# Isomorpfishm/SINGA

Hardware: AMD Instinct MI355X
Metric: protein-ligand graphs/sec GAN step (G+D fwd+bwd); scatter-TP kernel HBM GB/s (higher is better)
Workload: dtype f32

## Files before the change

### __graft_entry__.py

```python
import os
import subprocess
import sys

ROOT = os.path.dirname(os.path.abspath(__file__))
if ROOT not in sys.path:
    sys.path.insert(0, ROOT)

SRC = os.path.join(ROOT, "singa_amd", "csrc", "singa_hip.hip")
LIB = os.path.join(ROOT, "singa_amd", "lib", "libsinga_hip.so")


def build() -> None:
    os.makedirs(os.path.dirname(LIB), exist_ok=True)
    deps = [SRC, os.path.join(ROOT, "singa_amd", "csrc", "so3_index.h"), os.path.join(ROOT, "include", "singa_hip.h"),
            os.path.join(ROOT, "include", "singa_hip_lab.h"), os.path.join(ROOT, "include", "singa_hip_gen.h"),
            os.path.join(ROOT, "include", "singa_hip_force.h"), os.path.join(ROOT, "include", "singa_hip_swor.h"),
            os.path.join(ROOT, "include", "singa_hip_stream.h"), os.path.join(ROOT, "include", "singa_hip_valence.h"),
            os.path.join(ROOT, "include", "singa_hip_beam.h"), os.path.join(ROOT, "include", "singa_hip_units.h"),
            os.path.join(ROOT, "include", "singa_hip_prefix.h"), os.path.join(ROOT, "include", "singa_hip_data.h")]
    if not os.path.exists(LIB) or any(os.path.getmtime(d) > os.path.getmtime(LIB) for d in deps):
        hipcc = os.environ.get("HIPCC", "/opt/rocm/bin/hipcc")
        cmd = [hipcc, "--offload-arch=gfx950", "-O3", "-std=c++17", "-shared", "-fPIC", "-o", LIB, SRC]
        subprocess.check_call(cmd)
    import torch
    import singa_amd
    from singa_amd import _capi
    _capi.bind(LIB)


def smoke() -> None:
    import numpy as np
    import torch

    build()
    from oracle import singa_oracle as O
    from singa_amd import graph as G
    from singa_amd.config import load_config
    from singa_amd.model.GAN import SINGA
    from tests.helpers import golden, state_from_spec

    assert torch.cuda.is_available(), "smoke() needs a GPU"
    L = 2
    dev = "cuda:0"
    sd = state_from_spec(f"singa_L{L}")
    z = golden(f"singa_L{L}_B3.npz")
    names = ["3wi2_4tpp", "4agq_5a7b", "5cp5_4nue"]
    batch = G.collate([G.load_npz(os.path.join(ROOT, "tests", "golden", f"graph_{n}.npz"), with_lap=False) for n in names])
    batch.nodes[G.PA]["lap_pe"], batch.nodes[G.LA]["lap_pe"] = torch.tensor(z["lap_p"]), torch.tensor(z["lap_l"])
    batch.extras["edge_rot_mat"] = {k: torch.tensor(z[f"rot_{k}"]) for k in ("pp", "ll", "lp")}
    batch.extras["knn"] = {G.PA: torch.tensor(z["knn_p"]), G.LA: torch.tensor(z["knn_l"])}
    batch = batch.to(dev)
    model = SINGA(load_config(lmax=L), device=dev)
    model.load_state_dict(sd, strict=False)
    model.eval()
    logits = model(batch)
    loss = torch.nn.functional.cross_entropy(logits, batch["ligand_data"]["smiIndices_tgt"].reshape(-1))
    loss.backward()
    torch.cuda.synchronize()
    og = O.collate([O.load_graph_npz(os.path.join(ROOT, "tests", "golden", f"graph_{n}.npz")) for n in names])
    rots = {k: torch.as_tensor(z[f"rot_{k}"]) for k in ("pp", "ll", "lp")}
    with torch.no_grad():
        ref = O.singa_forward(sd, og, rots, L, torch.as_tensor(z["knn_p"]), torch.as_tensor(z["knn_l"]),
                              torch.as_tensor(z["lap_p"]), torch.as_tensor(z["lap_l"]))
    err = float((logits.detach().cpu().double() - ref.double()).norm() / ref.double().norm())
    gn = float(torch.sqrt(sum((p.grad.double() ** 2).sum() for p in model.parameters() if p.grad is not None)))
    print(f"smoke: loss {float(loss):.6f} (reference {float(z['loss']):.6f}), logits rel err vs oracle {err:.2e}, "
          f"grad norm {gn:.4f} (reference {float(z['grad_total']):.4f})")
    assert err < 1e-4, err
    assert abs(gn - float(z["grad_total"])) < 1e-4 * float(z["grad_total"])


if __name__ == "__main__":
# ... 4 lines not shown
```

### singa_amd/_capi.py

```python
import ctypes as C

P = C.c_void_p
I32 = C.c_int
I64 = C.c_int64
F32 = C.c_float


class Seg(C.Structure):
    _fields_ = [("ptr", P), ("ld", I64), ("rows", C.c_int32)]


SegArr = Seg * 3


class Gemm(C.Structure):
    _fields_ = [("a", P), ("b", P), ("c", P), ("bias", P), ("lda", I64), ("ldb", I64), ("ldc", I64), ("I", C.c_int32),
                ("J", C.c_int32), ("R", C.c_int32), ("a_group", C.c_int32), ("b_group", C.c_int32), ("c_group", C.c_int32),
                ("a_group_ld", I64), ("b_group_ld", I64), ("c_group_ld", I64), ("c_split_stride", I64), ("mask", P),
                ("addend", P), ("relu", C.c_int32), ("asum", P), ("asum_stride", I64)]


class CGemm(C.Structure):
    _fields_ = [("a", P), ("b", P), ("c", P), ("lda", I64), ("ldb", I64), ("ldc", I64), ("a_im", I64), ("b_im", I64),
                ("c_im", I64), ("c_split_stride", I64), ("I", C.c_int32), ("J", C.c_int32), ("R", C.c_int32),
# ... 117 lines not shown
_SWOR_SIGS = {
    "singa_swor_noise_host": ([U64, P, P, P, I32, P, P, P], I32),
    "singa_swor_work": ([I32, I32], C.c_longlong),
    "singa_swor_expand": ([P, P, P, P, I32, I32, I32, I32, I32, F32, U64, P, I32] + [P] * 8 + [P], I32),
    "singa_swor_select": ([P, P, P, P, P, I32, I32, I32, I32, I32, I32, I32] + [P] * 13 + [P], I32),
    "singa_swor_follow": ([P] * 8 + [I32] * 6 + [I64] * 4 + [P], I32),
}
SWOR_EXPORTS = tuple(_SWOR_SIGS)

_STREAM_SIGS = {
    "singa_dec_self_attn_rows": ([P] * 10 + [I32, I32, P, F32, P], I32),
    "singa_sample_token_stream": ([P] * 6 + [I32, I32, I32, I32, I32, F32, I32, F32, I32, I32] + [P] * 7 + [P], I32),
    "singa_stream_refill": ([I32] * 8 + [P] * 8 + [P], I32),
    "singa_stream_refill_host": ([I32] * 8 + [P] * 8, I32),
}
STREAM_EXPORTS = tuple(_STREAM_SIGS)

_VALENCE_SIGS = {
    "singa_sample_token_valence": ([P] * 7 + [I32, I32, I32, I32, I32, F32, I32, F32, I32, I32] + [P] * 12 + [P], I32),
    "singa_valence_rule_host": ([P] * 5 + [I32] + [P] * 3, I32),
}
VALENCE_EXPORTS = tuple(_VALENCE_SIGS)

_BEAM_SIGS = {
    "singa_beam_work": ([I32, I32], C.c_longlong),
    "singa_beam_expand": ([P] * 5 + [I32] * 5 + [P] * 5 + [P], I32),
    "singa_beam_select": ([P] * 4 + [I32] * 7 + [P] * 18 + [P], I32),
}
BEAM_EXPORTS = tuple(_BEAM_SIGS)

_UNITS_SIGS = {
    "singa_edge_mlp_units_fwd": ([P] * 13 + [I32, I32, I32, I32, P], I32),
    "singa_edge_mlp_units_bwd": ([P] * 8 + [I32, I32, I32, P], I32),
}
UNITS_EXPORTS = tuple(_UNITS_SIGS)

_PREFIX_SIGS = {
    "singa_sample_token_stream_forced": ([P] * 7 + [I32, I32, I32, I32, I32, F32, I32, F32, I32, I32] + [P] * 10 + [P], I32),
    "singa_swor_expand_forced": ([P, P, P, P, I32, I32, I32, I32, I32, F32, U64, P, I32] + [P] * 9 + [P], I32),
    "singa_forced_beam_expand": ([P] * 5 + [I32] * 5 + [P] * 6 + [P], I32),
}
PREFIX_EXPORTS = tuple(_PREFIX_SIGS)


class CollateField(C.Structure):
    _fields_ = [("src", P), ("dst", P), ("axis", C.c_int32), ("width", C.c_int32), ("kind", C.c_int32), ("base_axis", C.c_int32)]


_DATA_SIGS = {
    "singa_collate_batch": ([P, I32, I32, P, P, P, C.POINTER(CollateField), I32, C.POINTER(I64), P], I32),
}
DATA_EXPORTS = tuple(_DATA_SIGS)


def bind(path):
    import torch
    lib = C.CDLL(path)
    for name, (args, res) in list(_SIGS.items()) + list(_LAB_SIGS.items()) + list(_GEN_SIGS.items()) + \
            list(_FORCE_SIGS.items()) + list(_SWOR_SIGS.items()) + list(_STREAM_SIGS.items()) + list(_VALENCE_SIGS.items()) + \
            list(_BEAM_SIGS.items()) + list(_UNITS_SIGS.items()) + list(_PREFIX_SIGS.items()) + list(_DATA_SIGS.items()):
        fn = getattr(lib, name)
        fn.argtypes = args
        fn.restype = res
    return lib


def segs(items):
    arr = SegArr()
    for i, (p, ld, rows) in enumerate(items):
        arr[i].ptr, arr[i].ld, arr[i].rows = p, ld, rows
    return arr, len(items)


def check(lib, code, what):
    if code != 0:
        raise RuntimeError(f"{what} failed ({code}): {lib.singa_last_error_string().decode()}")
```

### singa_amd/csrc/singa_hip.hip

```cpp
#include <hip/hip_runtime.h>
#include <hip/hip_ext.h>

#include <math.h>
#include <stdint.h>
#include <stdio.h>
#include <string.h>
#include <type_traits>

#include "../../include/singa_hip.h"
#include "../../include/singa_hip_lab.h"
#include "../../include/singa_hip_gen.h"
#include "../../include/singa_hip_force.h"
#include "../../include/singa_hip_swor.h"
#include "../../include/singa_hip_stream.h"
#include "../../include/singa_hip_valence.h"
#include "../../include/singa_hip_beam.h"
#include "../../include/singa_hip_units.h"
#include "../../include/singa_hip_prefix.h"
#include "../../include/singa_hip_data.h"
#include "so3_index.h"

namespace {

thread_local char g_err[256] = "ok";

int fail(int code, const char* msg) {
    snprintf(g_err, sizeof(g_err), "%s", msg);
    return code;
}

int check_launch(const char* what) {
    hipError_t e = hipGetLastError();
    if (e != hipSuccess) {
        snprintf(g_err, sizeof(g_err), "%s: %s", what, hipGetErrorString(e));
        return (int)e;
    }
    return SINGA_OK;
}

struct ProfRec {
    hipEvent_t a, b;
    int E, N, tag;
};
constexpr int PROF_CAP = 8192;
ProfRec g_prof[PROF_CAP];
int g_prof_n = 0;
bool g_prof_on = false;
unsigned long long* g_stamp_buf = nullptr;
int g_stamp_cap = 0;
__global__ void stamp_kernel(unsigned long long* dst) { *dst = (unsigned long long)wall_clock64(); }
int g_prof_edges_hint = 0;

#ifndef SINGA_KEEP_VGPR
#define SINGA_KEEP_VGPR(x) __asm__ volatile("" : "+v"(x))
#endif

#define SINGA_LAUNCH(tag_, E_, N_, kern, grid, block, st, ...)                                                   \
    do {                                                                                                          \
        if (g_prof_on && g_prof_n < PROF_CAP) {                                                                   \
            ProfRec& r_ = g_prof[g_prof_n++];                                                                     \
            (void)hipEventCreate(&r_.a);                                                                          \
            (void)hipEventCreate(&r_.b);                                                                          \
            r_.E = (E_);                                                                                          \
            r_.N = (N_);                                                                                          \
            r_.tag = (tag_);                                                                                      \
            hipExtLaunchKernelGGL(kern, grid, block, 0, (st), r_.a, r_.b, 0, __VA_ARGS__);                        \
        } else if (g_stamp_buf && 2 * (g_prof_n + 2) <= g_stamp_cap && g_prof_n + 1 < PROF_CAP) {                 \
            if (g_prof_n == 0) {                                                                                  \
                g_prof[0].a = g_prof[0].b = nullptr;                                                              \
                g_prof[0].E = g_prof[0].N = g_prof[0].tag = 0;                                                    \
// ... 859 lines not shown
#pragma unroll
        for (int h = 0; h < H; ++h) gn[h] = g[((long long)n * H + h) * F + f];
        const int beg = row_ptr[n], end = row_ptr[n + 1];
        for (int e = beg; e < end; e += 2) {
            const bool two = e + 1 < end;
            const int e1 = two ? e + 1 : e;
            const int j0 = col[e], j1 = col[e1];
            const float w0 = wv[(long long)e * F + f], w1 = wv[(long long)e1 * F + f];
            float t0[H], t1[H], gw0 = 0.f, gw1 = 0.f;
#pragma unroll
            for (int h = 0; h < H; ++h) {
                t0[h] = gn[h] * hv[((long long)j0 * H + h) * F + f];
                t1[h] = gn[h] * hv[((long long)j1 * H + h) * F + f];
            }
#pragma unroll
            for (int h = 0; h < H; ++h) {
                gw0 = fmaf(t0[h], alpha[(long long)e * H + h], gw0);
                gw1 = fmaf(t1[h], alpha[(long long)e1 * H + h], gw1);
            }
            const float p0 = quad_reduce4(t0[0] * w0, t0[1] * w0, t0[2] * w0, t0[3] * w0, f);
            const float p1 = quad_reduce4(t1[0] * w1, t1[1] * w1, t1[2] * w1, t1[3] * w1, f);
            if ((f & 15) == 0) {
                g_alpha[(long long)e * H + quarter] = p0;
                if (two) g_alpha[(long long)e1 * H + quarter] = p1;
            }
            g_wv[(long long)e * F + f] = gw0;
            if (two) g_wv[(long long)e1 * F + f] = gw1;
        }
    }
}

template <int H>
__global__ void __launch_bounds__(64) gather_wsum_bwd_col_kernel(const float* __restrict__ g, const float* __restrict__ alpha,
                                                                 const float* __restrict__ wv, const int* __restrict__ col_ptr,
                                                                 const int* __restrict__ eperm, const int* __restrict__ row,
                                                                 float* __restrict__ g_hv, int N) {
    constexpr int F = 64;
    const int f = threadIdx.x;
    SINGA_XCD_NODE_LOOP(j, N) {
        float acc[H];
#pragma unroll
        for (int h = 0; h < H; ++h) acc[h] = 0.f;
        const int beg = col_ptr[j], end = col_ptr[j + 1];
        for (int i = beg; i < end; ++i) {
            const int e = eperm[i];
            const int n = row[e];
            const float w = wv[(long long)e * F + f];
#pragma unroll
            for (int h = 0; h < H; ++h)
                acc[h] = fmaf(alpha[(long long)e * H + h] * w, g[((long long)n * H + h) * F + f], acc[h]);
        }
#pragma unroll
        for (int h = 0; h < H; ++h) g_hv[((long long)j * H + h) * F + f] = acc[h];
    }
}


template <int C>
__device__ __forceinline__ void ln_row(const float* __restrict__ x, long long r, float (&xh)[C], float& rstd, float eps) {
    float mean = 0.f;
#pragma unroll
    for (int c = 0; c < C; c += 4) {
        const float4 v = *reinterpret_cast<const float4*>(x + r * C + c);
        xh[c] = v.x, xh[c + 1] = v.y, xh[c + 2] = v.z, xh[c + 3] = v.w;
        mean += (v.x + v.y) + (v.z + v.w);
    }
    mean *= 1.f / C;
    float var = 0.f;
#pragma unroll
    for (int c = 0; c < C; ++c) {
        xh[c] -= mean;
        var = fmaf(xh[c], xh[c], var);
    }
    rstd = 1.f / sqrtf(var * (1.f / C) + eps);
#pragma unroll
    for (int c = 0; c < C; ++c) xh[c] *= rstd;
}

template <int C>
__global__ void __launch_bounds__(64) ln_silu_fwd_kernel(const float* __restrict__ x, const float* __restrict__ gamma,
                                                         const float* __restrict__ beta, float* __restrict__ out, long long M,
                                                         float eps) {
    const long long stride = (long long)gridDim.x * 64;
    for (long long r = (long long)blockIdx.x * 64 + threadIdx.x; r < M; r += stride) {
        float xh[C], rstd;
        ln_row<C>(x, r, xh, rstd, eps);
        float o[C];
#pragma unroll
        for (int c = 0; c < C; ++c) {
            const float y = fmaf(xh[c], gamma[c], beta[c]);
            o[c] = y / (1.f + expf(-y));
        }
#pragma unroll
        for (int c = 0; c < C; c += 4) *reinterpret_cast<float4*>(out + r * C + c) = make_float4(o[c], o[c + 1], o[c + 2], o[c + 3]);
    }
}

template <int C>
__global__ void __launch_bounds__(64) ln_silu_bwd_kernel(const float* __restrict__ x, const float* __restrict__ gamma,
                                                         const float* __restrict__ beta, const float* __restrict__ g_out,
                                                         float* __restrict__ g_x, float* __restrict__ part, long long M,
                                                         float eps) {
    const long long tid = (long long)blockIdx.x * 64 + threadIdx.x, stride = (long long)gridDim.x * 64;
    float ag[C], ab[C];
#pragma unroll
    for (int c = 0; c < C; ++c) ag[c] = ab[c] = 0.f;
// ... 5300 lines not shown
                                                       g_out, gx, g_gate, EC, G));
    return check_launch("s2act_bwd");
}

int singa_edge_logits_fwd(const float* qp, const float* wk, const float* hk, const float* cterm, const int32_t* row_ptr,
                          const int32_t* col, float* qk, int N, int H, int D, float scale, void* stream) {
    if (!qp || !wk || !hk || !cterm || !row_ptr || !col || !qk) return fail(SINGA_E_NULL, "edge_logits_fwd: null pointer");
    if (H != 4 || D != 32) return fail(SINGA_E_SHAPE, "edge_logits: built for H = 4 heads, D = 32 key channels per head");
    if (N <= 0) return SINGA_OK;
    hipLaunchKernelGGL((edge_logits_fwd_kernel<32, 4>), dim3(kn_grid(N)), dim3(64), 0, (hipStream_t)stream, qp, wk,
                       hk, cterm, row_ptr, col, qk, N, scale);
    return check_launch("edge_logits_fwd");
}

int singa_edge_logits_bwd(const float* g, const float* qp, const float* wk, const float* hk, const int32_t* row_ptr,
                          const int32_t* col, const int32_t* col_ptr, const int32_t* eperm, const int32_t* row,
                          float* g_qp, float* g_wk, float* g_hk, float* g_cterm, int N, int H, int D, float scale,
                          void* stream) {
    if (!g || !qp || !wk || !hk || !row_ptr || !col || !col_ptr || !eperm || !row || !g_qp || !g_wk || !g_hk || !g_cterm)
        return fail(SINGA_E_NULL, "edge_logits_bwd: null pointer");
    if (H != 4 || D != 32) return fail(SINGA_E_SHAPE, "edge_logits: built for H = 4 heads, D = 32 key channels per head");
    if (N <= 0) return SINGA_OK;
    hipLaunchKernelGGL((edge_logits_bwd_row_kernel<32, 4>), dim3(kn_grid(N)), dim3(64), 0, (hipStream_t)stream, g,
                       qp, wk, hk, row_ptr, col, g_qp, g_wk, g_cterm, N, scale);
    hipLaunchKernelGGL((edge_logits_bwd_col_kernel<32, 4>), dim3(kn_grid(N)), dim3(64), 0, (hipStream_t)stream, g,
                       qp, wk, col_ptr, eperm, row, g_hk, N, scale);
    return check_launch("edge_logits_bwd");
}

int singa_gather_wsum_fwd(const float* alpha, const float* wv, const float* hv, const int32_t* row_ptr, const int32_t* col,
                          float* out, int N, int H, int F, void* stream) {
    if (!alpha || !wv || !hv || !row_ptr || !col || !out) return fail(SINGA_E_NULL, "gather_wsum_fwd: null pointer");
    if (H != 4 || F != 64) return fail(SINGA_E_SHAPE, "gather_wsum: built for H = 4 heads, F = 64 value channels per head");
    if (N <= 0) return SINGA_OK;
    hipLaunchKernelGGL((gather_wsum_fwd_kernel<4>), dim3(kn_grid(N)), dim3(64), 0, (hipStream_t)stream, alpha, wv,
                       hv, row_ptr, col, out, N);
    return check_launch("gather_wsum_fwd");
}

int singa_gather_wsum_bwd(const float* g, const float* alpha, const float* wv, const float* hv, const int32_t* row_ptr,
                          const int32_t* col, const int32_t* col_ptr, const int32_t* eperm, const int32_t* row,
                          float* g_alpha, float* g_wv, float* g_hv, int N, int H, int F, void* stream) {
    if (!g || !alpha || !wv || !hv || !row_ptr || !col || !col_ptr || !eperm || !row || !g_alpha || !g_wv || !g_hv)
        return fail(SINGA_E_NULL, "gather_wsum_bwd: null pointer");
    if (H != 4 || F != 64) return fail(SINGA_E_SHAPE, "gather_wsum: built for H = 4 heads, F = 64 value channels per head");
    if (N <= 0) return SINGA_OK;
    hipLaunchKernelGGL((gather_wsum_bwd_row_kernel<4>), dim3(kn_grid(N)), dim3(64), 0, (hipStream_t)stream, g,
                       alpha, wv, hv, row_ptr, col, g_alpha, g_wv, N);
    hipLaunchKernelGGL((gather_wsum_bwd_col_kernel<4>), dim3(kn_grid(N)), dim3(64), 0, (hipStream_t)stream, g,
                       alpha, wv, col_ptr, eperm, row, g_hv, N);
    return check_launch("gather_wsum_bwd");
}

#define SINGA_DISPATCH_S2SEP(lmax, edge, ...)                                                            \
    do {                                                                                                 \
        if (edge) {                                                                                      \
            constexpr bool EDGE_ = true; constexpr int C_ = 128;                                         \
            switch (lmax) {                                                                              \
                case 2: { constexpr int L_ = 2; __VA_ARGS__; } break;                                    \
                case 4: { constexpr int L_ = 4; __VA_ARGS__; } break;                                    \
                case 6: { constexpr int L_ = 6; __VA_ARGS__; } break;                                    \
                default: return fail(SINGA_E_LMAX, "s2act_sep: lmax must be 2, 4 or 6");                 \
            }                                                                                            \
        } else {                                                                                         \
            constexpr bool EDGE_ = false; constexpr int C_ = 512;                                        \
            switch (lmax) {                                                                              \
                case 2: { constexpr int L_ = 2; __VA_ARGS__; } break;                                    \
                case 4: { constexpr int L_ = 4; __VA_ARGS__; } break;                                    \
                case 6: { constexpr int L_ = 6; __VA_ARGS__; } break;                                    \
                default: return fail(SINGA_E_LMAX, "s2act_sep: lmax must be 2, 4 or 6");                 \
            }                                                                                            \
        }                                                                                                \
    } while (0)

int singa_s2act_sep_fwd(const singa_seg_t* x, int nseg, const float* gate, int64_t ldg, const float* P, const float* Q,
                        const float* A, float* out, int E, int C, int lmax, void* stream) {
    Segs s;
    if (!pack(x, nseg, &s) || !gate || !P || !Q || !A || !out) return fail(SINGA_E_NULL, "s2act_sep_fwd: null pointer");
    const bool edge = nseg == 3;
    if (!(edge && C == 128) && !(nseg == 1 && C == 512))
        return fail(SINGA_E_SHAPE, "s2act_sep: built for (3 segments, C = 128) and (1 segment, C = 512)");
    if (edge && (s.rows[0] != lmax + 1 || s.rows[1] != 2 * lmax || s.rows[2] != 2 * (lmax - 1)))
        return fail(SINGA_E_SHAPE, "s2act_sep(edge): segment rows must be L+1, 2L, 2(L-1)");
    if (!edge && s.rows[0] != (lmax + 1) * (lmax + 1)) return fail(SINGA_E_SHAPE, "s2act_sep(node): rows must be (L+1)^2");
    if (E <= 0) return SINGA_OK;
    long long EC = (long long)E * C;
    int blocks = (int)((EC + 255) / 256);
    const int tag = edge ? SINGA_PROF_S2_EDGE_FWD : SINGA_PROF_S2_NODE_FWD;
    bool pair = (((uintptr_t)gate | (uintptr_t)out) & 7) == 0 && ldg % 2 == 0 && (edge || lmax <= 4);
    for (int i = 0; i < nseg; ++i) pair = pair && ((uintptr_t)s.p[i] & 7) == 0 && s.ld[i] % 2 == 0;
    if (pair) {
        const long long EC2 = EC / 2;
        blocks = (int)((EC2 + 255) / 256);
        SINGA_DISPATCH_S2SEP(lmax, edge, SINGA_LAUNCH(tag, E, 0, (s2act_sep_fwd2_kernel<L_, EDGE_, C_>), dim3(blocks), dim3(256),
                                                      (hipStream_t)stream, s, gate, (long long)ldg, P, Q, out, EC2));
        return check_launch("s2act_sep_fwd");
    }
    SINGA_DISPATCH_S2SEP(lmax, edge, SINGA_LAUNCH(tag, E, 0, (s2act_sep_fwd_kernel<L_, EDGE_, C_>), dim3(blocks), dim3(256),
                                                  (hipStream_t)stream, s, gate, (long long)ldg, P, Q, A, out, EC));
    return check_launch("s2act_sep_fwd");
}

int singa_s2act_sep_bwd_seg(const singa_seg_t* x, int nseg, const float* gate, int64_t ldg, const float* P, const float* Q,
                            const float* A, const float* g_out, const singa_seg_mut_t* gx, float* g_gate, int64_t ld_gg, int E,
                            int C, int lmax, void* stream) {
    Segs s;
// ... 1383 lines not shown
```

### singa_amd/model/CProMG.py

```python
import math
import os

import numpy as np
import torch
import torch.nn as nn
import torch.nn.functional as F
from torch.nn import BatchNorm1d, Conv1d, Dropout, Embedding, LayerNorm, Sequential

from .. import ops
from ..nn import Linear


class ShiftedSoftplus(nn.Module):
    def __init__(self, device="cuda"):
        super().__init__()
        self.shift = math.log(2.0)

    def forward(self, x):
        return F.softplus(x) - self.shift


class GaussianSmearing(nn.Module):
    def __init__(self, start=0.0, stop=10.0, num_gaussians=50, device="cuda"):
        super().__init__()
# ... 68 lines not shown
                  else torch.zeros((), dtype=torch.bool, device=dev))
        n_groups, last, triple = torch.stack([gid[-1] + 1, skey[-1], triple.to(gid.dtype)]).tolist()
        n_edges = n_groups - (1 if last == sentinel else 0)
        ukey = torch.zeros(n_groups, dtype=torch.int64, device=dev).scatter_(0, gid, skey)[:n_edges]
        ln2 = torch.cat([ln, ln])[perm]
        if not triple:
            nxt = torch.cat([ln2[1:], ln2[-1:]])
            prv = torch.cat([ln2[:1], ln2[:-1]])
            has_next = torch.cat([~new[1:], new.new_zeros(1)])
            mean = torch.where(new, torch.where(has_next, 0.5 * (ln2 + nxt), ln2), 0.5 * (prv + ln2))
            ln = torch.zeros(n_groups, device=dev).scatter_(0, gid, mean)[:n_edges]
        else:
            cnt = torch.zeros(n_groups, device=dev).index_add_(0, gid, torch.ones_like(ln2))[:n_edges]
            ln = torch.zeros(n_groups, device=dev).index_add_(0, gid, ln2)[:n_edges] / cnt
        row, col = ukey // N, ukey % N
        fused = ln.is_cuda and smear.offset.numel() == 64
        ea = None if fused else smear(ln)
        self.n_edges = n_edges + N
        if cap is not None:
            extra = cap - self.n_edges
            nd = N - n_real
            if extra < 0 or nd < 2:
                raise OverflowError(f"KnnEdges: {self.n_edges} edges do not fit the capacity {cap}")
            i = torch.arange(extra, device=dev)
            ps = (i * nd) // max(extra, 1)
            row = torch.cat([row, n_real + ps])
            col = torch.cat([col, n_real + (ps + 1 + i % (nd - 1)) % nd])
            if not fused:
                ea = torch.cat([ea, ea.new_zeros(extra, ea.shape[1])])
        loop = torch.arange(N, device=dev)
        bounds = torch.arange(N + 1, device=dev)
        if ln.is_cuda:
            E0 = row.shape[0]
            seg_ptr = torch.searchsorted(row, bounds)
            order = torch.empty(E0 + N, dtype=torch.int64, device=dev)
            order[torch.arange(E0, device=dev) + row] = torch.arange(E0, device=dev)
            order[seg_ptr[1:] + loop] = E0 + loop
            row, col = torch.cat([row, loop]), torch.cat([col, loop])
            self.row, self.col = row[order], col[order]
            seg32 = seg_ptr.to(torch.int32)
            if fused:
                self.attr = ops.knn_edge_attr(ln, seg32, E0, n_edges, smear.offset, smear.coeff)
            else:
                deg = ops.segment_sum_rows(ea.contiguous(), seg32)
                self.attr = torch.cat([-ea, deg], 0)[order].contiguous()
        else:
            deg = torch.zeros(N, ea.shape[1], device=dev).index_add_(0, row, ea)
            row, col = torch.cat([row, loop]), torch.cat([col, loop])
            attr = torch.cat([-ea, deg], 0)
            order = torch.argsort(row, stable=True)
            self.row, self.col, self.attr = row[order], col[order], attr[order].contiguous()
        self.row_ptr = torch.searchsorted(self.row, bounds).to(torch.int32)
        self.row32, self.col32 = self.row.to(torch.int32), self.col.to(torch.int32)
        eperm = torch.argsort(self.col32 if ln.is_cuda else self.col, stable=True)
        self.eperm = eperm.to(torch.int32)
        self.col_ptr = torch.searchsorted(self.col[eperm], bounds).to(torch.int32)
        self.N = N
        self.unit_a, self.unit_b = self._units(ukey, n_real, bool(triple))

    def _units(self, ukey, n_real, repeats):
        row, col = self.row, self.col
        E, N = row.shape[0], self.N
        idx = torch.arange(E, device=row.device)
        if repeats or ukey.numel() == 0:
            single = torch.ones_like(row, dtype=torch.bool)
        else:
            single = row == col
            if n_real is not None:
                single |= torch.maximum(row, col) >= n_real
        mate = torch.where(single, idx, torch.searchsorted(ukey, col * N + row) + col)
        first = single | (row < col)
        slot = torch.where(first, torch.cumsum(first, 0) - 1, E)
        both = torch.stack([idx, mate], 1).to(torch.int32)
        units = torch.full((E + 1, 2), -1, dtype=torch.int32, device=row.device).index_copy_(0, slot, both)
        return units[:E, 0].contiguous(), units[:E, 1].contiguous()

    def tensors(self):
        return [self.row, self.col, self.attr, self.row_ptr, self.row32, self.col32, self.eperm, self.col_ptr, self.unit_a,
                self.unit_b]


class MultiHeadAttention(nn.Module):

    def __init__(self, hidden_channels, edge_channels, key_channels, num_heads=1, device="cuda"):
        super().__init__()
        assert hidden_channels % num_heads == 0 and key_channels % num_heads == 0
        self.num_heads = num_heads
        self.k_lin = Conv1d(hidden_channels, key_channels, 1, groups=num_heads, bias=False, device=device)
        self.q_lin = Conv1d(hidden_channels, key_channels, 1, groups=num_heads, bias=False, device=device)
        self.v_lin = Conv1d(hidden_channels, hidden_channels, 1, groups=num_heads, bias=False, device=device)
        kh, vh = key_channels // num_heads, hidden_channels // num_heads
        self.weight_k_net = Sequential(Linear(edge_channels, kh, device=device), ShiftedSoftplus(), Linear(kh, kh, device=device))
        self.weight_k_lin = Linear(kh, kh, device=device)
        self.weight_v_net = Sequential(Linear(edge_channels, vh, device=device), ShiftedSoftplus(), Linear(vh, vh, device=device))
        self.weight_v_lin = Linear(vh, vh, device=device)
        self.centroid_lin = Linear(hidden_channels, hidden_channels, device=device)
        self.act = ShiftedSoftplus()
        self.out_transform = Linear(hidden_channels, hidden_channels, device=device)
        self.layer_norm = LayerNorm(hidden_channels, device=device)

    def _edge_mlp(self, net, x):
        return net[2](ops.bias_ssp(ops.linear(x, net[0].weight), net[0].bias))

    def forward(self, node_attr, edges: KnnEdges):
        N = node_attr.size(0)
        h_keys, h_queries, h_values = ops.grouped_linear3(node_attr, self.k_lin.weight, self.q_lin.weight, self.v_lin.weight,
                                                          self.num_heads)
        scale = 1.0 / math.sqrt(h_keys.size(-1))
        if edges.attr.shape[1] == 64 and self.weight_k_net[0].out_features == 32 and self.weight_v_net[0].out_features == 64:
            W_k, W_v = ops.edge_mlp_pair(edges.attr, (self.weight_k_net[0], self.weight_k_net[2]),
                                         (self.weight_v_net[0], self.weight_v_net[2]),
                                         units=(edges.unit_a, edges.unit_b))
        else:
            W_k = self._edge_mlp(self.weight_k_net, edges.attr)
            W_v = self._edge_mlp(self.weight_v_net, edges.attr)
        qp = ops.linear_nn(h_queries, self.weight_k_lin.weight)
        cterm = ops.rowdot_bias(h_queries, self.weight_k_lin.bias, scale)
        qk_ij = ops.edge_logits(qp, W_k, h_keys, cterm, edges, scale)
        alpha = ops.segment_softmax(qk_ij, edges.row_ptr, 0.0)
        S = ops.gather_wsum(alpha, W_v, h_values, edges)
        aggr_msg = ops.linear(S, self.weight_v_lin.weight, self.weight_v_lin.bias).view(N, -1)
        out = ops.bias_ssp(ops.linear_add(node_attr, self.centroid_lin.weight, None, aggr_msg), self.centroid_lin.bias)
        return ops.layer_norm_residual(self.out_transform(out), None, self.layer_norm)


def _dense_attention(module, Q, K, V, attn_mask, key_channels, hidden_channels):
    B, heads = Q.size(0), module.num_heads
    dk, dv = key_channels // heads, hidden_channels // heads
    scale = 1.0 / math.sqrt(dk)
    if dk == 32 and dv == 64:
        WQ, WK, WV = ((m.weight, m.bias) for m in (module.W_Q, module.W_K, module.W_V))
        if Q is K and K is V:
# ... 296 lines not shown
```

### singa_amd/ops.py

```python
import ctypes
import math
import warnings

import torch

warnings.filterwarnings("ignore", message=".*preferred_blas_library is an experimental feature.*")

from . import _capi, _lib, so3


PROFILE_ON = False


def profile_start(in_graph=False):
    global PROFILE_ON, _STAMPS
    PROFILE_ON = True
    if in_graph:
        _STAMPS = torch.zeros(2 * 8192 + 2, dtype=torch.int64, device="cuda")
        _chk(_lib.lib().singa_prof_stamps(_p(_STAMPS), _STAMPS.numel()), "singa_prof_stamps")
    else:
        _chk(_lib.lib().singa_prof_enable(1), "singa_prof_enable")


_STAMPS = None
# ... 568 lines not shown
        L, eps = ctx.L, ctx.eps
        N, K, C = x.shape
        lib = _lib.lib()
        if gy is None:
            return gskip, None, None, None, None
        gy = gy.contiguous()
        nparts = lib.singa_so3_rmsnorm_nparts(N)
        gx = torch.empty_like(x)
        gwp = torch.empty(nparts, (L + 1) * C, device=x.device, dtype=torch.float32)
        gbp = torch.empty(nparts, C, device=x.device, dtype=torch.float32)
        if gskip is not None:
            gskip = gskip.contiguous()
            _chk(lib.singa_so3_rmsnorm_bwd_add(_p(x), _p(weight), _p(gy), _p(gskip), _p(gx), _p(gwp), _p(gbp), N, C, L, eps,
                                               _stream()), "singa_so3_rmsnorm_bwd_add")
        else:
            _chk(lib.singa_so3_rmsnorm_bwd(_p(x), _p(weight), _p(gy), _p(gx), _p(gwp), _p(gbp), N, C, L, eps, _stream()),
                 "singa_so3_rmsnorm_bwd")
        gw = param_colsum(gwp, [(0, (L + 1) * C, ctx.params[0])])[0]
        if gw is not None:
            gw = gw.view(L + 1, C)
        return gx, gw, param_colsum(gbp, [(0, C, ctx.params[1])])[0], None, None


def so3_rmsnorm_skip(x, weight, bias, L, eps=1e-5):
    return _SO3RMSNormSkip.apply(x, weight, bias, L, eps)


class _EdgeLogits(torch.autograd.Function):
    @staticmethod
    def forward(ctx, qp, wk, hk, cterm, edges, scale):
        qp, wk, hk, cterm = qp.contiguous(), wk.contiguous(), hk.contiguous(), cterm.contiguous()
        _dev(qp, wk, hk, cterm)
        N, H, D = qp.shape
        qk = torch.empty(wk.shape[0], H, device=qp.device, dtype=torch.float32)
        ctx.edges, ctx.scale = edges, scale
        if wk.shape[0] == 0:
            ctx.save_for_backward(qp, wk, hk)
            return qk
        _chk(_lib.lib().singa_edge_logits_fwd(_p(qp), _p(wk), _p(hk), _p(cterm), _p(edges.row_ptr), _p(edges.col32),
                                              _p(qk), N, H, D, scale, _stream()), "singa_edge_logits_fwd")
        ctx.save_for_backward(qp, wk, hk)
        ctx.edges, ctx.scale = edges, scale
        return qk

    @staticmethod
    def backward(ctx, g):
        qp, wk, hk = ctx.saved_tensors
        e, N, H, D = ctx.edges, qp.shape[0], qp.shape[1], qp.shape[2]
        g = g.contiguous()
        g_qp, g_wk, g_hk = torch.empty_like(qp), torch.empty_like(wk), torch.empty_like(hk)
        g_c = torch.empty(N, H, device=g.device, dtype=torch.float32)
        if wk.shape[0] == 0:
            return g_qp.zero_(), g_wk, g_hk.zero_(), g_c.zero_(), None, None
        _chk(_lib.lib().singa_edge_logits_bwd(_p(g), _p(qp), _p(wk), _p(hk), _p(e.row_ptr), _p(e.col32), _p(e.col_ptr),
                                              _p(e.eperm), _p(e.row32), _p(g_qp), _p(g_wk), _p(g_hk), _p(g_c), N, H, D,
                                              ctx.scale, _stream()), "singa_edge_logits_bwd")
        return g_qp, g_wk, g_hk, g_c, None, None


def edge_logits(qp, wk, hk, cterm, edges, scale):
    return _EdgeLogits.apply(qp, wk, hk, cterm, edges, scale)


class _GatherWSum(torch.autograd.Function):
    @staticmethod
    def forward(ctx, alpha, wv, hv, edges):
        alpha, wv, hv = alpha.contiguous(), wv.contiguous(), hv.contiguous()
        _dev(alpha, wv, hv)
        N, H, F = hv.shape
        out = torch.empty(N, H, F, device=hv.device, dtype=torch.float32)
        ctx.edges = edges
        if alpha.shape[0] == 0:
            ctx.save_for_backward(alpha, wv, hv)
            return out.zero_()
        _chk(_lib.lib().singa_gather_wsum_fwd(_p(alpha), _p(wv), _p(hv), _p(edges.row_ptr), _p(edges.col32), _p(out), N,
                                              H, F, _stream()), "singa_gather_wsum_fwd")
        ctx.save_for_backward(alpha, wv, hv)
        ctx.edges = edges
        return out

    @staticmethod
    def backward(ctx, g):
        alpha, wv, hv = ctx.saved_tensors
        e = ctx.edges
        N, H, F = hv.shape
        g = g.contiguous()
        g_a, g_wv, g_hv = torch.empty_like(alpha), torch.empty_like(wv), torch.empty_like(hv)
        if alpha.shape[0] == 0:
            return g_a, g_wv, g_hv.zero_(), None
        _chk(_lib.lib().singa_gather_wsum_bwd(_p(g), _p(alpha), _p(wv), _p(hv), _p(e.row_ptr), _p(e.col32), _p(e.col_ptr),
                                              _p(e.eperm), _p(e.row32), _p(g_a), _p(g_wv), _p(g_hv), N, H, F, _stream()),
             "singa_gather_wsum_bwd")
        return g_a, g_wv, g_hv, None


def gather_wsum(alpha, wv, hv, edges):
    return _GatherWSum.apply(alpha, wv, hv, edges)


class _LnSilu(torch.autograd.Function):
    @staticmethod
    def forward(ctx, x, gamma, beta, eps):
        ctx.params = (gamma, beta)
        x, gamma, beta = x.contiguous(), gamma.contiguous(), beta.contiguous()
        _dev(x, gamma, beta)
        C = x.shape[-1]
        M = x.numel() // C
        out = torch.empty_like(x)
        _chk(_lib.lib().singa_ln_silu_fwd(_p(x), _p(gamma), _p(beta), _p(out), M, C, eps, _stream()), "singa_ln_silu_fwd")
        ctx.save_for_backward(x, gamma, beta)
        ctx.eps = eps
        return out

    @staticmethod
    def backward(ctx, g):
        x, gamma, beta = ctx.saved_tensors
        g = g.contiguous()
        C = x.shape[-1]
        M = x.numel() // C
        lib = _lib.lib()
        gx = torch.empty_like(x)
        part = torch.empty(lib.singa_ln_silu_nparts(M), 2 * C, device=x.device, dtype=torch.float32)
        _chk(lib.singa_ln_silu_bwd(_p(x), _p(gamma), _p(beta), _p(g), _p(gx), _p(part), M, C, ctx.eps, _stream()),
             "singa_ln_silu_bwd")
        gg, gb = param_colsum(part, [(0, C, ctx.params[0]), (C, C, ctx.params[1])])
        return gx, gg, gb, None


def ln_silu(x, gamma, beta, eps=1e-5):
    return _LnSilu.apply(x, gamma, beta, eps)


def dec_layer_step(x, w, k_cache, v_cache, pos, cross_k, cross_v, pad, beams, per_row=False):
    _dev(x, k_cache, v_cache, cross_k, cross_v)
    lib, st = _lib.lib(), _stream()
    R, P, S = x.shape[0], k_cache.shape[2], cross_v.shape[2]
    y, z, out = torch.empty_like(x), torch.empty_like(x), torch.empty_like(x)
    a, c, f = w["self"], w["cross"], w["ffn"]
    if per_row:
        _check_views("dec_layer_step", ((pos, torch.int64, (R,)),))
    self_attn, name = (lib.singa_dec_self_attn_rows, "singa_dec_self_attn_rows") if per_row else \
        (lib.singa_dec_self_attn, "singa_dec_self_attn")
# ... 1396 lines not shown
```

Before: 886.2.

## Use reverse-edge mates to fuse column-side gradients into row-pass attention backward

For symmetric graphs without repeated edges, each edge's reverse edge (mate) is recorded. The attention-logit and weighted-gather backward kernels can then compute the column-side gradients (g_hk, g_hv) in the same row-ordered pass instead of a separate column-sorted traversal. This also skips building the column permutation and col_ptr when mates exist. The cost is extra gathers of mate-indexed gradients and alpha, plus new kernels hardcoded for H=4, D=32 and F=64. Correctness depends on the graph being exactly symmetric.

```diff
diff --git a/__graft_entry__.py b/__graft_entry__.py
--- a/__graft_entry__.py
+++ b/__graft_entry__.py
@@ -17,7 +17,8 @@
             os.path.join(ROOT, "include", "singa_hip_force.h"), os.path.join(ROOT, "include", "singa_hip_swor.h"),
             os.path.join(ROOT, "include", "singa_hip_stream.h"), os.path.join(ROOT, "include", "singa_hip_valence.h"),
             os.path.join(ROOT, "include", "singa_hip_beam.h"), os.path.join(ROOT, "include", "singa_hip_units.h"),
-            os.path.join(ROOT, "include", "singa_hip_prefix.h"), os.path.join(ROOT, "include", "singa_hip_data.h")]
+            os.path.join(ROOT, "include", "singa_hip_prefix.h"), os.path.join(ROOT, "include", "singa_hip_data.h"),
+            os.path.join(ROOT, "include", "singa_hip_mates.h")]
     if not os.path.exists(LIB) or any(os.path.getmtime(d) > os.path.getmtime(LIB) for d in deps):
         hipcc = os.environ.get("HIPCC", "/opt/rocm/bin/hipcc")
         cmd = [hipcc, "--offload-arch=gfx950", "-O3", "-std=c++17", "-shared", "-fPIC", "-o", LIB, SRC]
diff --git a/include/singa_hip_mates.h b/include/singa_hip_mates.h
--- /dev/null
+++ b/include/singa_hip_mates.h
@@ -0,0 +1,17 @@
+#ifndef SINGA_HIP_MATES_H
+#define SINGA_HIP_MATES_H
+#include <stdint.h>
+#ifdef __cplusplus
+extern "C" {
+#endif
+int singa_edge_logits_bwd_mates(const float* g, const float* qp, const float* wk, const float* hk, const int32_t* row_ptr,
+                                const int32_t* col, const int32_t* mate, float* g_qp, float* g_wk, float* g_hk, float* g_cterm,
+                                int N, int H, int D, float scale, void* stream);
+
+int singa_gather_wsum_bwd_mates(const float* g, const float* alpha, const float* wv, const float* hv, const int32_t* row_ptr,
+                                const int32_t* col, const int32_t* mate, float* g_alpha, float* g_wv, float* g_hv, int N, int H,
+                                int F, void* stream);
+#ifdef __cplusplus
+}
+#endif
+#endif
diff --git a/singa_amd/_capi.py b/singa_amd/_capi.py
--- a/singa_amd/_capi.py
+++ b/singa_amd/_capi.py
@@ -193,13 +193,20 @@
 }
 DATA_EXPORTS = tuple(_DATA_SIGS)
 
+_MATES_SIGS = {
+    "singa_edge_logits_bwd_mates": ([P] * 11 + [I32, I32, I32, F32, P], I32),
+    "singa_gather_wsum_bwd_mates": ([P] * 10 + [I32, I32, I32, P], I32),
+}
+MATES_EXPORTS = tuple(_MATES_SIGS)
+
 
 def bind(path):
     import torch
     lib = C.CDLL(path)
     for name, (args, res) in list(_SIGS.items()) + list(_LAB_SIGS.items()) + list(_GEN_SIGS.items()) + \
             list(_FORCE_SIGS.items()) + list(_SWOR_SIGS.items()) + list(_STREAM_SIGS.items()) + list(_VALENCE_SIGS.items()) + \
-            list(_BEAM_SIGS.items()) + list(_UNITS_SIGS.items()) + list(_PREFIX_SIGS.items()) + list(_DATA_SIGS.items()):
+            list(_BEAM_SIGS.items()) + list(_UNITS_SIGS.items()) + list(_PREFIX_SIGS.items()) + list(_DATA_SIGS.items()) + \
+            list(_MATES_SIGS.items()):
         fn = getattr(lib, name)
         fn.argtypes = args
         fn.restype = res
diff --git a/singa_amd/csrc/singa_hip.hip b/singa_amd/csrc/singa_hip.hip
--- a/singa_amd/csrc/singa_hip.hip
+++ b/singa_amd/csrc/singa_hip.hip
@@ -16,6 +16,7 @@
 #include "../../include/singa_hip_valence.h"
 #include "../../include/singa_hip_beam.h"
 #include "../../include/singa_hip_units.h"
+#include "../../include/singa_hip_mates.h"
 #include "../../include/singa_hip_prefix.h"
 #include "../../include/singa_hip_data.h"
 #include "so3_index.h"
@@ -981,6 +982,160 @@
         }
 #pragma unroll
         for (int h = 0; h < H; ++h) g_hv[((long long)j * H + h) * F + f] = acc[h];
+    }
+}
+
+template <int D, int H>
+__global__ void __launch_bounds__(64) edge_logits_bwd_mates_kernel(const float* __restrict__ g, const float* __restrict__ qp,
+                                                                   const float* __restrict__ wk, const float* __restrict__ hk,
+                                                                   const int* __restrict__ row_ptr, const int* __restrict__ col,
+                                                                   const int* __restrict__ mate, float* __restrict__ g_qp,
+                                                                   float* __restrict__ g_wk, float* __restrict__ g_hk,
+                                                                   float* __restrict__ g_cterm, int N, float scale) {
+    constexpr int SL = 64 / D;
+    const int lane = threadIdx.x, d = lane % D, slot = lane / D;
+    const int E = row_ptr[N];
+    SINGA_XCD_NODE_LOOP(n, N) {
+        float q[H], aq[H], ac[H], ak[H];
+#pragma unroll
+        for (int h = 0; h < H; ++h) {
+            q[h] = qp[((long long)n * H + h) * D + d] * scale;
+            aq[h] = 0.f;
+            ac[h] = 0.f;
+            ak[h] = 0.f;
+        }
+        const int beg = row_ptr[n], end = row_ptr[n + 1];
+        for (int e0 = beg; e0 < end; e0 += 2 * SL) {
+            const int ea = e0 + slot, eb = e0 + SL + slot;
+            const bool oka = ea < end, okb = eb < end;
+            const int sa = oka ? ea : beg, sb = okb ? eb : beg;
+            const int ja = col[sa], jb = col[sb];
+            const int ma = mate[sa], mb = mate[sb];
+            const bool va = oka && ma >= 0 && ma < E, vb = okb && mb >= 0 && mb < E;
+            const float wa = wk[(long long)sa * D + d], wb = wk[(long long)sb * D + d];
+            const long long xa = va ? ma : sa, xb = vb ? mb : sb;
+            float gea[H], geb[H], gma[H], gmb[H];
+#pragma unroll
+            for (int h = 0; h < H; ++h) {
+                gea[h] = g[(long long)sa * H + h];
+                geb[h] = g[(long long)sb * H + h];
+                gma[h] = g[xa * H + h];
+                gmb[h] = g[xb * H + h];
+            }
+            float ka[H], kb[H], pa[H], pb[H];
+#pragma unroll
+            for (int h = 0; h < H; ++h) {
+                ka[h] = hk[((long long)ja * H + h) * D + d];
+                kb[h] = hk[((long long)jb * H + h) * D + d];
+                pa[h] = qp[((long long)ja * H + h) * D + d];
+                pb[h] = qp[((long long)jb * H + h) * D + d];
+            }
+            if (oka) {
+                float gw = 0.f;
+#pragma unroll
+                for (int h = 0; h < H; ++h) {
+                    aq[h] = fmaf(gea[h] * wa, ka[h], aq[h]);
+                    gw = fmaf(gea[h] * q[h], ka[h], gw);
+                    ac[h] += gea[h];
+                }
+                g_wk[(long long)ea * D + d] = gw;
+            }
+            if (va) {
+#pragma unroll
+                for (int h = 0; h < H; ++h) ak[h] = fmaf(gma[h] * wa, pa[h], ak[h]);
+            }
+            if (okb) {
+                float gw = 0.f;
+#pragma unroll
+                for (int h = 0; h < H; ++h) {
+                    aq[h] = fmaf(geb[h] * wb, kb[h], aq[h]);
+                    gw = fmaf(geb[h] * q[h], kb[h], gw);
+                    ac[h] += geb[h];
+                }
+                g_wk[(long long)eb * D + d] = gw;
+            }
+            if (vb) {
+#pragma unroll
+                for (int h = 0; h < H; ++h) ak[h] = fmaf(gmb[h] * wb, pb[h], ak[h]);
+            }
+        }
+#pragma unroll
+        for (int h = 0; h < H; ++h) {
+            float a = aq[h], c = ac[h], k = ak[h];
+            for (int o = D; o < 64; o <<= 1) {
+                a += __shfl_xor(a, o, 64);
+                c += __shfl_xor(c, o, 64);
+                k += __shfl_xor(k, o, 64);
+            }
+            if (slot == 0) {
+                g_qp[((long long)n * H + h) * D + d] = a * scale;
+                g_hk[((long long)n * H + h) * D + d] = k * scale;
+            }
+            if (lane == 0) g_cterm[(long long)n * H + h] = c;
+        }
+    }
+}
+
+template <int H>
+__global__ void __launch_bounds__(64) gather_wsum_bwd_mates_kernel(const float* __restrict__ g, const float* __restrict__ alpha,
+                                                                   const float* __restrict__ wv, const float* __restrict__ hv,
+                                                                   const int* __restrict__ row_ptr, const int* __restrict__ col,
+                                                                   const int* __restrict__ mate, float* __restrict__ g_alpha,
+                                                                   float* __restrict__ g_wv, float* __restrict__ g_hv, int N) {
+    static_assert(H == 4, "the four-way folded reduction is written for four heads");
+    constexpr int F = 64;
+    const int f = threadIdx.x, quarter = f >> 4;
+    const int E = row_ptr[N];
+    SINGA_XCD_NODE_LOOP(n, N) {
+        float gn[H], acc[H];
+#pragma unroll
+        for (int h = 0; h < H; ++h) {
+            gn[h] = g[((long long)n * H + h) * F + f];
+            acc[h] = 0.f;
+        }
+        const int beg = row_ptr[n], end = row_ptr[n + 1];
+        for (int e = beg; e < end; e += 2) {
+            const bool two = e + 1 < end;
+            const int e1 = two ? e + 1 : e;
+            const int j0 = col[e], j1 = col[e1];
+            const int m0 = mate[e], m1 = mate[e1];
+            const bool v0 = m0 >= 0 && m0 < E, v1 = two && m1 >= 0 && m1 < E;
+            const int s0 = v0 ? m0 : e, s1 = v1 ? m1 : e1;
+            const float w0 = wv[(long long)e * F + f], w1 = wv[(long long)e1 * F + f];
+            float t0[H], t1[H], c0[H], c1[H], a0[H], a1[H], gw0 = 0.f, gw1 = 0.f;
+#pragma unroll
+            for (int h = 0; h < H; ++h) {
+                t0[h] = gn[h] * hv[((long long)j0 * H + h) * F + f];
+                t1[h] = gn[h] * hv[((long long)j1 * H + h) * F + f];
+                c0[h] = g[((long long)j0 * H + h) * F + f];
+                c1[h] = g[((long long)j1 * H + h) * F + f];
+                a0[h] = alpha[(long long)s0 * H + h];
+                a1[h] = alpha[(long long)s1 * H + h];
+            }
+#pragma unroll
+            for (int h = 0; h < H; ++h) {
+                gw0 = fmaf(t0[h], alpha[(long long)e * H + h], gw0);
+                gw1 = fmaf(t1[h], alpha[(long long)e1 * H + h], gw1);
+            }
+            const float p0 = quad_reduce4(t0[0] * w0, t0[1] * w0, t0[2] * w0, t0[3] * w0, f);
+            const float p1 = quad_reduce4(t1[0] * w1, t1[1] * w1, t1[2] * w1, t1[3] * w1, f);
+            if ((f & 15) == 0) {
+                g_alpha[(long long)e * H + quarter] = p0;
+                if (two) g_alpha[(long long)e1 * H + quarter] = p1;
+            }
+            g_wv[(long long)e * F + f] = gw0;
+            if (two) g_wv[(long long)e1 * F + f] = gw1;
+            if (v0) {
+#pragma unroll
+                for (int h = 0; h < H; ++h) acc[h] = fmaf(a0[h] * w0, c0[h], acc[h]);
+            }
+            if (v1) {
+#pragma unroll
+                for (int h = 0; h < H; ++h) acc[h] = fmaf(a1[h] * w1, c1[h], acc[h]);
+            }
+        }
+#pragma unroll
+        for (int h = 0; h < H; ++h) g_hv[((long long)n * H + h) * F + f] = acc[h];
     }
 }
 
@@ -6387,6 +6542,30 @@
     return check_launch("gather_wsum_bwd");
 }
 
+int singa_edge_logits_bwd_mates(const float* g, const float* qp, const float* wk, const float* hk, const int32_t* row_ptr,
+                                const int32_t* col, const int32_t* mate, float* g_qp, float* g_wk, float* g_hk, float* g_cterm,
+                                int N, int H, int D, float scale, void* stream) {
+    if (!g || !qp || !wk || !hk || !row_ptr || !col || !mate || !g_qp || !g_wk || !g_hk || !g_cterm)
+        return fail(SINGA_E_NULL, "edge_logits_bwd_mates: null pointer");
+    if (H != 4 || D != 32) return fail(SINGA_E_SHAPE, "edge_logits_bwd_mates: built for H = 4 heads, D = 32 key channels per head");
+    if (N <= 0) return SINGA_OK;
+    hipLaunchKernelGGL((edge_logits_bwd_mates_kernel<32, 4>), dim3(kn_grid(N)), dim3(64), 0, (hipStream_t)stream, g,
+                       qp, wk, hk, row_ptr, col, mate, g_qp, g_wk, g_hk, g_cterm, N, scale);
+    return check_launch("edge_logits_bwd_mates");
+}
+
+int singa_gather_wsum_bwd_mates(const float* g, const float* alpha, const float* wv, const float* hv, const int32_t* row_ptr,
+                                const int32_t* col, const int32_t* mate, float* g_alpha, float* g_wv, float* g_hv, int N, int H,
+                                int F, void* stream) {
+    if (!g || !alpha || !wv || !hv || !row_ptr || !col || !mate || !g_alpha || !g_wv || !g_hv)
+        return fail(SINGA_E_NULL, "gather_wsum_bwd_mates: null pointer");
+    if (H != 4 || F != 64) return fail(SINGA_E_SHAPE, "gather_wsum_bwd_mates: built for H = 4 heads, F = 64 value channels per head");
+    if (N <= 0) return SINGA_OK;
+    hipLaunchKernelGGL((gather_wsum_bwd_mates_kernel<4>), dim3(kn_grid(N)), dim3(64), 0, (hipStream_t)stream, g,
+                       alpha, wv, hv, row_ptr, col, mate, g_alpha, g_wv, g_hv, N);
+    return check_launch("gather_wsum_bwd_mates");
+}
+
 #define SINGA_DISPATCH_S2SEP(lmax, edge, ...)                                                            \
     do {                                                                                                 \
         if (edge) {                                                                                      \
diff --git a/singa_amd/model/CProMG.py b/singa_amd/model/CProMG.py
--- a/singa_amd/model/CProMG.py
+++ b/singa_amd/model/CProMG.py
@@ -144,11 +144,13 @@
             self.row, self.col, self.attr = row[order], col[order], attr[order].contiguous()
         self.row_ptr = torch.searchsorted(self.row, bounds).to(torch.int32)
         self.row32, self.col32 = self.row.to(torch.int32), self.col.to(torch.int32)
-        eperm = torch.argsort(self.col32 if ln.is_cuda else self.col, stable=True)
-        self.eperm = eperm.to(torch.int32)
-        self.col_ptr = torch.searchsorted(self.col[eperm], bounds).to(torch.int32)
         self.N = N
-        self.unit_a, self.unit_b = self._units(ukey, n_real, bool(triple))
+        self.unit_a, self.unit_b, self.mate = self._units(ukey, n_real, bool(triple))
+        self.eperm = self.col_ptr = None
+        if self.mate is None:
+            eperm = torch.argsort(self.col32 if ln.is_cuda else self.col, stable=True)
+            self.eperm = eperm.to(torch.int32)
+            self.col_ptr = torch.searchsorted(self.col[eperm], bounds).to(torch.int32)
 
     def _units(self, ukey, n_real, repeats):
         row, col = self.row, self.col
@@ -165,11 +167,12 @@
         slot = torch.where(first, torch.cumsum(first, 0) - 1, E)
         both = torch.stack([idx, mate], 1).to(torch.int32)
         units = torch.full((E + 1, 2), -1, dtype=torch.int32, device=row.device).index_copy_(0, slot, both)
-        return units[:E, 0].contiguous(), units[:E, 1].contiguous()
+        mate32 = None if repeats else torch.where(single & (row != col), -1, mate).to(torch.int32)
+        return units[:E, 0].contiguous(), units[:E, 1].contiguous(), mate32
 
     def tensors(self):
-        return [self.row, self.col, self.attr, self.row_ptr, self.row32, self.col32, self.eperm, self.col_ptr, self.unit_a,
-                self.unit_b]
+        by_col = [self.mate] if self.mate is not None else [self.eperm, self.col_ptr]
+        return [self.row, self.col, self.attr, self.row_ptr, self.row32, self.col32] + by_col + [self.unit_a, self.unit_b]
 
 
 class MultiHeadAttention(nn.Module):
diff --git a/singa_amd/ops.py b/singa_amd/ops.py
--- a/singa_amd/ops.py
+++ b/singa_amd/ops.py
@@ -644,6 +644,11 @@
         g_c = torch.empty(N, H, device=g.device, dtype=torch.float32)
         if wk.shape[0] == 0:
             return g_qp.zero_(), g_wk, g_hk.zero_(), g_c.zero_(), None, None
+        if getattr(e, "mate", None) is not None:
+            _chk(_lib.lib().singa_edge_logits_bwd_mates(_p(g), _p(qp), _p(wk), _p(hk), _p(e.row_ptr), _p(e.col32), _p(e.mate),
+                                                        _p(g_qp), _p(g_wk), _p(g_hk), _p(g_c), N, H, D, ctx.scale, _stream()),
+                 "singa_edge_logits_bwd_mates")
+            return g_qp, g_wk, g_hk, g_c, None, None
         _chk(_lib.lib().singa_edge_logits_bwd(_p(g), _p(qp), _p(wk), _p(hk), _p(e.row_ptr), _p(e.col32), _p(e.col_ptr),
                                               _p(e.eperm), _p(e.row32), _p(g_qp), _p(g_wk), _p(g_hk), _p(g_c), N, H, D,
                                               ctx.scale, _stream()), "singa_edge_logits_bwd")
@@ -680,6 +685,11 @@
         g_a, g_wv, g_hv = torch.empty_like(alpha), torch.empty_like(wv), torch.empty_like(hv)
         if alpha.shape[0] == 0:
             return g_a, g_wv, g_hv.zero_(), None
+        if getattr(e, "mate", None) is not None:
+            _chk(_lib.lib().singa_gather_wsum_bwd_mates(_p(g), _p(alpha), _p(wv), _p(hv), _p(e.row_ptr), _p(e.col32), _p(e.mate),
+                                                        _p(g_a), _p(g_wv), _p(g_hv), N, H, F, _stream()),
+                 "singa_gather_wsum_bwd_mates")
+            return g_a, g_wv, g_hv, None
         _chk(_lib.lib().singa_gather_wsum_bwd(_p(g), _p(alpha), _p(wv), _p(hv), _p(e.row_ptr), _p(e.col32), _p(e.col_ptr),
                                               _p(e.eperm), _p(e.row32), _p(g_a), _p(g_wv), _p(g_hv), N, H, F, _stream()),
              "singa_gather_wsum_bwd")
```

Result: faster. 896.7, median of 6 (+1.2%).
